# jwh97nn/AnyRef

Measured on AMD Instinct MI355X. Metric: images/sec (1024^2, 7B LLM+ViT-L+SAM-H), higher is better.
Workload: dtype bf16 (LLaMA / CLIP) + f16 (SAM encoder); 1 GPU; C2: LLaVA-7B + CLIP ViT-L/14 + SAM-H refer-seg forward, 1024x1024, S=320 prompt, 10 new tokens, KV cache; batch_per_gpu=1, global_batch=1, parallelism=dp1, weights=random-init N(0,0.02^2) rounded to bf16

## Files before the change

### anyref_amd/_lib.py

```python
from __future__ import annotations

import ctypes as C
import os

import torch

HERE = os.path.dirname(os.path.abspath(__file__))
LIB_PATH = os.path.join(HERE, "libanyref_hip.so")

ABI_VERSION = 2
F32, BF16, F16 = 0, 1, 2
MODE_PARITY, MODE_PERF, MODE_PERF_FP8W, MODE_PARITY16, MODE_PERF_F16 = 0, 1, 2, 3, 4


class AnyrefConfig(C.Structure):
    _fields_ = [
        ("abi_version", C.c_int32), ("mode", C.c_int32),
        ("clip_image", C.c_int32), ("clip_patch", C.c_int32), ("clip_dim", C.c_int32),
        ("clip_heads", C.c_int32), ("clip_layers_run", C.c_int32), ("clip_mlp", C.c_int32),
        ("clip_eps", C.c_float),
        ("llm_vocab", C.c_int32), ("llm_dim", C.c_int32), ("llm_heads", C.c_int32),
        ("llm_layers", C.c_int32), ("llm_mlp", C.c_int32), ("llm_max_seq", C.c_int32),
        ("llm_rms_eps", C.c_float), ("llm_rope_theta", C.c_float),
        ("sam_img", C.c_int32), ("sam_patch", C.c_int32), ("sam_dim", C.c_int32), ("sam_depth", C.c_int32),
# ... 36 lines not shown
    "anyref_set_overlap": (_I, [_P, _I]),
    "anyref_set_early_tail": (_I, [_P, _I]),
    "anyref_set_extra_event": (_I, [_P, _P]),
    "anyref_set_graphs": (_I, [_P, _I]),
    "anyref_set_side_share": (_I, [_P, _I, _I]),
    "anyref_profile_enable": (_I, [_P, _I]),
    "anyref_profile_config": (_I, [_P, C.c_char_p, _I]),
    "anyref_profile_collect": (_I, [_P]),
    "anyref_profile_calibrate": (_I, [_P, _P, C.POINTER(C.c_double)]),
    "anyref_profile_read": (_I, [_P, _I, C.c_char_p, _I, C.POINTER(C.c_double), C.POINTER(_L),
                                C.POINTER(C.c_double), C.POINTER(C.c_double)]),
    "anyref_stamps_enable": (_I, [_P, _I]),
    "anyref_stamps_collect": (_I, [_P, C.POINTER(_L)]),
    "anyref_stamps_dropped": (_I, [_P, C.POINTER(_L)]),
    "anyref_stamps_read": (_I, [_P, _L, C.c_char_p, _I, C.POINTER(C.c_double), C.POINTER(C.c_double),
                               C.POINTER(C.c_double), C.POINTER(_I)]),
    "anyref_stamps_spread": (_I, [_P, _L, C.POINTER(C.c_double), C.POINTER(C.c_double), C.POINTER(C.c_double)]),
    "anyref_device_bytes": (_L, [_P]),
    "anyref_mode_name": (C.c_char_p, [_P]),
    "anyref_inexact_weights": (_I, [_P, C.POINTER(_L)]),
    "anyref_op_gemm": (_I, [_I, _P, _P, _P, _P, _P, _P, _P, _I, _I, _I, _I, _I]),
    "anyref_op_gemm_fp8": (_I, [_P, _P, _P, _P, _P, _P, _P, _I, _I, _I, _I, _I]),
    "anyref_op_quant_fp8": (_I, [_P, _P, _I, _I, _P, _P]),
    "anyref_op_gemv_fp8": (_I, [_P, _P, _P, _F, _P, _P, _P, _P, _P, _P, _I, _I, _I]),
    "anyref_op_iou_counts": (_I, [_P, _P, _P, _I, _L, _P]),
    "anyref_op_avs_counts": (_I, [_P, _P, _P, _I, _L, _P, _I, _F, _P, _P]),
    "anyref_op_sam_preprocess": (_I, [_P, _P, _I, _I, _I, C.POINTER(C.c_float), C.POINTER(C.c_float), _P]),
    "anyref_op_pil_resample_u8": (_I, [_P, _P, _I, _I, _I, _P, _P, _I, _I, _P, _P, _I, _P, _P, _I]),
    "anyref_op_pool_ref_tokens": (_I, [_P, _P, _I, _I, _I, _I, _P]),
    "anyref_op_kaldi_fbank": (_I, [_P, _P, _I, _I, _I, _I, _I, C.c_float, _P, _I, _P, _P, _I, C.c_float, C.c_float, _P]),
    "anyref_op_clip_finish": (_I, [_P, _P, _I, _I, _I, _I, _I, _I, _I, C.POINTER(C.c_float), C.POINTER(C.c_float), _P]),
    "anyref_op_gemv": (_I, [_I, _P, _P, _P, _F, _P, _P, _P, _P, _P, _I, _I, _I, _I]),
    "anyref_op_gemv_xn": (_I, [_I, _P, _P, _P, _F, _P, _P, _P, _P, _P, _I, _I, _I, _I, _P, _P, _I]),
    "anyref_op_rope_table": (_I, [_I, _I, _F, _P]),
    "anyref_op_decode_attn": (_I, [_I, _P, _P, _I, _I, _I, _P, _P, _P, _P, _I, _F, _P, _P, _I]),
    "anyref_op_rope_cache": (_I, [_I, _P, _P, _P, _P, _I, _I, _I, _I, _P, _P, _P, _P, _P, _P, _I, _P]),
    "anyref_op_argmax": (_I, [_P, _P, _I, _I, _I, _P, _P, _P, _I, _I, _I, _P, _P, _P]),
    "anyref_op_norm": (_I, [_I, _P, _P, _P, _P, _P, _I, _I, _F, _I]),
    "anyref_op_attention": (_I, [_I, _P, _P, _P, _P, _P, _I, _I, _I, _I, _I, _F, _I, _P, _P, _P, _I, _I]),
    "anyref_op_attention_tab": (_I, [_I, _P, _P, _P, _P, _P, _I, _I, _I, _I, _F, _P, _P, _I, _I, _I]),
    "anyref_op_gemm_gather": (_I, [_I, _P, _P, _P, _P, _P, _P, _P, _I, _I, _I, _I]),
    "anyref_op_attention_relp": (_I, [_I, _P, _P, _P, _P, _P, _I, _I, _I, _I, _F, _P, _I, _I, _I]),
    "anyref_op_rel_pos": (_I, [_I, _P, _P, _P, _P, _I, _I, _I, _I, _P, _P]),
    "anyref_op_postprocess": (_I, [_P, _P, _I, _I, _I, _I, _I, _I, _I, _I, _P]),
    "anyref_op_last_error": (C.c_char_p, []),
}

_lib = None


def load() -> C.CDLL:
    global _lib
    if _lib is not None:
        return _lib
    if not os.path.exists(LIB_PATH):
        raise RuntimeError(
            f"{LIB_PATH} not found: build the HIP backend first "
            "(`python -c 'import __graft_entry__ as g; g.build()'` or `make -C anyref_amd/csrc`). "
            "anyref_amd has no CPU fallback.")
    lib = C.CDLL(LIB_PATH)
    for name, (res, args) in SYMBOLS.items():
        fn = getattr(lib, name)
        fn.restype = res
        fn.argtypes = args
    _lib = lib
    return lib
# ... 1 lines not shown
```

### anyref_amd/csrc/gemv.hip

```cpp
#include <cstdlib>
#include <stdexcept>
#include <type_traits>

#include "kernels.h"

namespace anyref {

static bool gemv_pair_knob() {
  static const bool p = !(getenv("ANYREF_GEMV_PAIR") && atoi(getenv("ANYREF_GEMV_PAIR")) == 0);
  return p;
}
static int gemv_grid_knob() {
  static const int g = getenv("ANYREF_GEMV_GRID") ? atoi(getenv("ANYREF_GEMV_GRID")) : 0;
  return g;
}

#ifndef ANYREF_GEMV_NO_DOT2
#define ANYREF_GEMV_NO_DOT2 0
#endif
constexpr bool NO_DOT2 = ANYREF_GEMV_NO_DOT2;
template <typename T, int NB, bool DUAL, int XPT, bool W8 = false, bool PAIR = false>
__global__ __launch_bounds__(512) void gemv_kernel(GemvArgs a, int b0, int nb) {
  static_assert(!W8 || std::is_same<T, bf16>::value, "fp8 weights go with bf16 activations");
  using WE = std::conditional_t<is_split<T>::value, bf16, T>;
  using XE = std::conditional_t<is_split<T>::value, float, T>;
  using WT = std::conditional_t<W8, uint8_t, WE>;
  constexpr int VN = W8 ? 16 : Vec16<WE>::N;
  constexpr int R = DUAL ? 1 : 2;
  constexpr int RW = 2;
  constexpr int UNR = 4;
  constexpr bool DOT2 = (std::is_same<T, bf16>::value || is_half16<T>::value) && !W8 && !NO_DOT2;
  extern __shared__ __attribute__((aligned(16))) char smem[];
  XE* xs = reinterpret_cast<XE*>(smem);
  __shared__ float red[NB][8];
  __shared__ float red2[2][4][2][NB];
  const int tid = threadIdx.x, lane = tid & 63, wave = tid >> 6;
  const int K = a.K;
  __shared__ unsigned long long st_t[2];
  __shared__ unsigned st_cnt;
  unsigned long long t_begin = 0;
  if (a.stamp.base) {
    t_begin = wall_clock64();
    if (tid == 0) {
      st_t[0] = ~0ull;
      st_t[1] = 0;
      st_cnt = 0;
    }
// ... 173 lines not shown
      const int n0 = (unit + (t / nchp) * nunits) * R;
#pragma unroll
      for (int r = 0; r < RW; ++r)
#pragma unroll
        for (int b = 0; b < NB; ++b) acc[r][b] = wave_sum(acc[r][b]);
      if constexpr (PAIR) {
        const int buf = (t / nchp) & 1;
        if (half == 1 && lane == 0) {
#pragma unroll
          for (int r = 0; r < RW; ++r)
#pragma unroll
            for (int b = 0; b < NB; ++b) red2[buf][wave >> 1][r][b] = acc[r][b];
        }
        __syncthreads();
        if (half == 0) {
#pragma unroll
          for (int r = 0; r < RW; ++r)
#pragma unroll
            for (int b = 0; b < NB; ++b) acc[r][b] += red2[buf][wave >> 1][r][b];
        }
      }
      if (lane < R * NB && half == 0) {
        const int r = lane / NB, b = lane % NB, n = n0 + r;
        float v = 0.f, v2 = 0.f;
#pragma unroll
        for (int rr = 0; rr < R; ++rr)
#pragma unroll
          for (int bb = 0; bb < NB; ++bb)
            if (lane == rr * NB + bb) {
              v = acc[rr][bb];
              v2 = DUAL ? acc[RW - 1][bb] : 0.f;
            }
        if (n < a.N && b < nb) {
          if constexpr (W8) {
            v *= a.wscale[(int64_t)n * a.ws_stride];
            if (DUAL) v2 *= a.wscale2[(int64_t)n * a.ws_stride];
          }
          if (a.bias) v += a.bias[n];
          if (DUAL)
            v = apply_act(v, ACT_SILU) * v2;
          else
            v = apply_act(v, a.act);
          const int64_t o = (int64_t)(b0 + b) * a.ldy + n;
          if (a.resid) v += a.resid[o];
          a.y[o] = v;
        }
      }
#pragma unroll
      for (int r = 0; r < RW; ++r)
#pragma unroll
        for (int b = 0; b < NB; ++b) acc[r][b] = 0.f;
    }
    if (t + 1 < items) {
#pragma unroll
      for (int u = 0; u < UNR; ++u)
#pragma unroll
        for (int r = 0; r < RW; ++r) wcur[u][r] = wnxt[u][r];
    }
  }
  if (a.stamp.base && lane == 0) {
    atomicMin(&st_t[0], t_begin);
    atomicMax(&st_t[1], (unsigned long long)wall_clock64());
    if (atomicAdd(&st_cnt, 1u) == 7u) {
      const int e = *a.stamp.epoch;
      if (e < a.stamp.max_epoch) {
        unsigned long long* p = a.stamp.base + (size_t)e * a.stamp.stride + (size_t)blockIdx.x * 2;
        p[0] = st_t[0];
        p[1] = st_t[1];
      }
    }
  }
}


template <bool W8, bool DUAL, int XV>
__global__ __launch_bounds__(512) void gemv_rows8_kernel(GemvArgs a, int b0, int nb, int kh0, int rs) {
  typedef __attribute__((ext_vector_type(2))) __bf16 bf16x2;
  constexpr int NB = 8, UNR = 8;
  constexpr int EPL = W8 ? 16 : 8;
  constexpr int SEG = 16 * EPL;
  constexpr int CH = UNR * SEG;
  using WT = std::conditional_t<W8, uint8_t, bf16>;
  extern __shared__ __attribute__((aligned(16))) char smem[];
  __shared__ float red[NB][8];
  const int tid = threadIdx.x, lane = tid & 63, wave = tid >> 6;
  const int j = lane & 3, q = lane >> 2;
  const int K = a.K;
  const int ldw = a.ldw > 0 ? a.ldw : K;
  const WT* __restrict__ W = reinterpret_cast<const WT*>(a.W);
  const WT* __restrict__ W2 = reinterpret_cast<const WT*>(a.W2);
  constexpr int R = DUAL ? 2 : 4;
  const int ngroups = cdiv(a.N, R);
  const int nwaves = gridDim.x * 8, gw = blockIdx.x * 8 + wave;
  const int my_groups = gw < ngroups ? (ngroups - gw + nwaves - 1) / nwaves : 0;
  const int nkh = kh0 < K ? 2 : 1;
  const int nch0 = cdiv(kh0, CH), nch1 = nkh == 2 ? cdiv(K - kh0, CH) : 0;
  const int items0 = my_groups * nch0, items = items0 + my_groups * nch1;
  const int pl = rs > 0 ? (rs - 64) / 2 : 0;
  uint4v w0[UNR], w1[UNR], w2[UNR];
  auto item_pos = [&](int t, int& g, int& kbeg, int& kend) __attribute__((always_inline)) {
    int gi, c;
    if (t < items0) {
      gi = t / nch0; c = t - gi * nch0;
      kbeg = c * CH; kend = kh0;
// ... 231 lines not shown
  const int rs = cdiv(kh0 * 2, 256) * 256 + 64;
  const size_t lds = (size_t)8 * rs;
  const int grid = 256;
  const double wbytes = (double)a.N * a.K * wsz * (dual ? 2 : 1) + (double)nb * (a.K + a.N) * 4;
  char tag[48];
  snprintf(tag, sizeof(tag), "gemv_rows8_%s%s", w8 ? "fp8w" : "bf16", dual ? "_swiglu" : "");
  ProfScope prof(tag, 2.0 * nb * a.N * (double)a.K * (dual ? 2 : 1), wbytes, s);
  auto launch = [&](auto w8_t, auto dual_t, auto xv_t) {
    constexpr bool W8 = decltype(w8_t)::value, DUAL = decltype(dual_t)::value;
    constexpr int XV = decltype(xv_t)::value;
    auto kern = &gemv_rows8_kernel<W8, DUAL, XV>;
    static KernelAttrOnce once;
    ensure_dyn_lds(once, reinterpret_cast<const void*>(kern), 152 * 1024);
    hipLaunchKernelGGL(kern, dim3(grid), dim3(512), lds, s, a, b0, nb, kh0, rs);
  };
  using TT = std::true_type;
  using FF = std::false_type;
  using X2 = std::integral_constant<int, 2>;
  using X3 = std::integral_constant<int, 3>;
  auto by_xv = [&](auto w8_t, auto dual_t) {
    if (a.gain && a.K > 4096) launch(w8_t, dual_t, X3());
    else launch(w8_t, dual_t, X2());
  };
  if (w8) {
    if (dual) by_xv(TT(), TT());
    else by_xv(TT(), FF());
  } else {
    if (dual) by_xv(FF(), TT());
    else by_xv(FF(), FF());
  }
  return true;
}

template <typename T, int NB>
static void gemv_dispatch(const GemvArgs& a_in, int b0, int nb, hipStream_t s) {
  GemvArgs a = a_in;
  const size_t lds = (size_t)NB * a.K * (is_split<T>::value ? 4 : sizeof(T));
  if (lds > 150 * 1024) throw std::runtime_error("gemv: K too large for the LDS activation stage");
  int grid = 256 * (lds > 76 * 1024 ? 1 : 2);
  const int grid_rule = grid;
  if (a.grid > 0 && a.grid < grid) grid = a.grid;
  if (gemv_grid_knob() > 0) grid = gemv_grid_knob();
  auto go = [&](auto xpt_tag) {
    constexpr int XPT = decltype(xpt_tag)::value;
    const double wsz = a.w_fp8 ? 1.0 : (is_split<T>::value ? 2.0 : (double)sizeof(T));
    const double wbytes = (double)a.N * a.K * wsz * (a.W2 ? 2 : 1) + (double)nb * (a.K + a.N) * 4;
    char tag[40];
    snprintf(tag, sizeof(tag), "gemv_%s%s_x%d",
             a.w_fp8 ? "fp8w" : (is_split<T>::value ? "sp16" : is_half16<T>::value ? "f16" : sizeof(T) == 2 ? "bf16" : "f32"),
             a.W2 ? "_swiglu" : "", XPT);
    ProfScope prof(tag, 2.0 * nb * a.N * (double)a.K * (a.W2 ? 2 : 1), wbytes, s);
    if (g_stamp && g_stamp->on) a.stamp = g_stamp->slot(tag, wbytes, grid);
    auto launch = [&](auto dual_t, auto w8_t, auto pair_t) {
      constexpr bool DUAL = decltype(dual_t)::value, W8 = decltype(w8_t)::value, PAIR = decltype(pair_t)::value;
      auto kern = &gemv_kernel<T, NB, DUAL, XPT, W8, PAIR>;
      static KernelAttrOnce once;
      ensure_dyn_lds(once, reinterpret_cast<const void*>(kern), 150 * 1024);
      hipLaunchKernelGGL(kern, dim3(grid), dim3(512), lds, s, a, b0, nb);
    };
    using TT = std::true_type;
    using FF = std::false_type;
    const bool pair = gemv_pair_knob() && cdiv(a.N, a.W2 ? 1 : 2) * 2 <= (gemv_grid_knob() > 0 ? grid : grid_rule) * 8;
    auto by_pair = [&](auto dual_t, auto w8_t) {
      if (pair) launch(dual_t, w8_t, TT());
      else launch(dual_t, w8_t, FF());
    };
    if constexpr (std::is_same<T, bf16>::value) {
      if (a.w_fp8) {
        if (a.W2) by_pair(TT(), TT());
        else by_pair(FF(), TT());
        return;
      }
    }
    if (a.W2) by_pair(TT(), FF());
    else by_pair(FF(), FF());
  };
  if (a.K <= 512 * 8)
    go(std::integral_constant<int, 8>());
  else if (a.K <= 512 * 24)
    go(std::integral_constant<int, 24>());
  else if (a.K <= 512 * 32)
    go(std::integral_constant<int, 32>());
  else
    throw std::runtime_error("gemv: K > 16384 not supported");
}

template <typename T>
void launch_gemv(const GemvArgs& a, hipStream_t s) {
  const int VN = a.w_fp8 ? 16 : Vec16<std::conditional_t<is_split<T>::value, bf16, T>>::N;
  if (a.K % VN || ((uintptr_t)a.W & 15)) throw std::runtime_error("gemv: K must be a multiple of 16 bytes");
  if (a.w_fp8 && (!std::is_same<T, bf16>::value || !a.wscale || (a.W2 && !a.wscale2)))
    throw std::runtime_error("gemv: fp8 weights need the bf16 mode and per-row scales");
  if (((uintptr_t)a.x & 15) || a.ldx % 4 || a.K % 4 || (a.gain && ((uintptr_t)a.gain & 15)) ||
      (a.xn_out && (((uintptr_t)a.xn_out & 15) || a.xn_ld % 4)))
    throw std::runtime_error("gemv: x / gain / xn_out rows must be 16-byte aligned");
// ... 47 lines not shown
```

### anyref_amd/csrc/kernels.h

```cpp
#pragma once
#include <cstdlib>
#include <map>
#include <string>
#include <utility>
#include <vector>

#include "common.h"

namespace anyref {

struct ProfStat {
  double ms = 0;
  int64_t count = 0;
  double flops = 0, bytes = 0;
};
class Profiler {
 public:
  ~Profiler();
  bool begin(const char* tag, double flops, double bytes, hipStream_t s);
  void end(hipStream_t s);
  void collect();
  void reset();
  void calibrate(hipStream_t s);
  double null_ms = 0.0;
// ... 99 lines not shown
  float* slabs_out = nullptr;
  int slabs = 0;
  bool* norm_done = nullptr;
  int batch = 1;
  int64_t sA = 0, sW = 0, sC = 0, sR = 0, sBias = 0;
};
template <typename T>
void launch_gemm(const GemmArgs& a, hipStream_t s);
void gemm_reserve_workspace(hipStream_t s, size_t bytes);
void gemm_release_workspace(hipStream_t s);
void attn_release_workspace(hipStream_t s);

struct GemvArgs {
  const float* x = nullptr;
  const float* gain = nullptr;
  float eps = 1e-6f;
  const void* W = nullptr;
  const void* W2 = nullptr;
  const float* bias = nullptr;
  float* y = nullptr;
  const float* resid = nullptr;
  int B = 1, N = 0, K = 0, ldx = 0, ldy = 0;
  int act = ACT_NONE;
  int ldw = 0;
  int w_fp8 = 0;
  const float* wscale = nullptr;
  const float* wscale2 = nullptr;
  int ws_stride = 1;
  float* xn_out = nullptr;
  const int* xn_row_map = nullptr;
  int xn_ld = 0;
  StampArgs stamp;
  int grid = 0;
};
template <typename T>
void launch_gemv(const GemvArgs& a, hipStream_t s);
void launch_gemv_skinny_f32(const GemvArgs& a, hipStream_t s);
void launch_quant_fp8_rows(const float* src, int lds, int N, int K, uint8_t* q, int ldq, float* scale, hipStream_t s,
                           int scale_stride = 1, unsigned long long* inexact = nullptr);
void launch_dequant_fp8_rows(const uint8_t* q, int ldq, const float* scale, int N, int K, void* out_bf16, int ldo,
                             hipStream_t s);

struct NormArgs {
  const float* x = nullptr;
  const float* gain = nullptr;
  const float* bias = nullptr;
  void* y = nullptr;
  const int* row_map = nullptr;
  int M = 0, D = 0, ldx = 0, ldy = 0;
  float eps = 1e-5f;
  int rms = 0;
  int y_f32 = 0;
  int act = ACT_NONE;
  void* fill_dst = nullptr;
  int fill_ld = 0, fill_n = 0, fill_N = 0;
  const int* fill_rows = nullptr;
  const float* fill_bias = nullptr;
  bool* fill_done = nullptr;
};
template <typename T>
void launch_norm(const NormArgs& a, hipStream_t s);

struct AttnArgs {
  const void *Q = nullptr, *K = nullptr, *V = nullptr;
  void* O = nullptr;
  int64_t q_bs = 0, q_rs = 0, q_hs = 0;
  int64_t k_bs = 0, k_rs = 0, k_hs = 0;
// ... 127 lines not shown
```

### anyref_amd/csrc/model.hip

```cpp
#include <algorithm>
#include <cmath>
#include <cstdlib>
#include <cstring>
#include <type_traits>

#include "model.h"

namespace anyref {

ModelBase::ModelBase(const anyref_config& c, int device) : cfg(c), device_(device) { HIP_TRY(hipSetDevice(device)); }

ModelBase::~ModelBase() {
  (void)hipSetDevice(device_);
  (void)hipDeviceSynchronize();
  for (auto& kv : allocs_) (void)hipFree(kv.first);
  if (wcount_) (void)hipFree(wcount_);
}

unsigned long long* ModelBase::weight_counts() {
  if (!wcount_) {
    HIP_TRY(hipMalloc(&wcount_, 2 * sizeof(unsigned long long)));
    HIP_TRY(hipMemset(wcount_, 0, 2 * sizeof(unsigned long long)));
  }
  return wcount_;
// ... 198 lines not shown
  bool gemm(hipStream_t s, const E* A, int lda, const Lin<typename ModeTypes<E>::W>& l, void* C, int ldc, int M, int act, bool c_f32,
            const float* resid = nullptr, int ldr = 0, const int* row_map = nullptr, const Affine* nrm = nullptr,
            void* nrm_out = nullptr, bool swiglu = false, float ln_eps = -1.f, const int* a_row_map = nullptr) {
    GemmArgs a;
    bool fused = false;
    a.swiglu_pairs = swiglu ? 1 : 0;
    if (nrm && nrm_out) {
      a.norm_gain = nrm->g; a.norm_out = nrm_out; a.norm_ld = l.n; a.norm_eps = cfg.llm_rms_eps; a.norm_done = &fused;
      if (ln_eps >= 0.f) {
        a.norm_bias = nrm->b;
        a.norm_eps = ln_eps;
      }
    }
    a.A = A; a.lda = apad<E>(lda); a.W = l.w; a.ldw = l.stride(); a.bias = l.b; a.C = C; a.ldc = c_f32 ? ldc : apad<E>(ldc);
    a.M = M; a.N = l.n;
    a.norm_ld = apad<E>(a.norm_ld);
    a.K = l.k; a.act = act; a.c_f32 = c_f32 ? 1 : 0; a.resid = resid; a.ldr = ldr; a.row_map = row_map;
    a.a_row_map = a_row_map;
    a.max_wg = cap_wg_;
    if constexpr (std::is_same<E, T>::value && !SPT) {
      if (l.w8) {
        if (l.k % 64 == 0) {
          a.W = l.w8; a.w_fp8 = 1; a.col_scale = l.ws;
        } else {
          launch_dequant_fp8_rows(l.w8, l.stride(), l.ws, l.n, l.k, deq_buf_, l.k, s);
          a.W = deq_buf_; a.ldw = l.k;
        }
      }
    }
    launch_gemm<E>(a, s);
    return fused;
  }
  int gemv_grid_ = 0;
  void gemv_w(GemvArgs& g, const Lin<W>& l, int row0 = 0) const {
    g.ldw = l.stride();
    g.grid = gemv_grid_;
    if (l.w8) {
      g.W = l.w8 + (size_t)row0 * l.stride();
      g.wscale = l.ws + row0;
      g.w_fp8 = 1;
    } else {
      g.W = l.w + (size_t)row0 * l.stride();
    }
  }
  void gemv_w2(GemvArgs& g, const Lin<W>& l, int row0) const {
    if (l.w8) {
      g.W2 = l.w8 + (size_t)row0 * l.stride();
      g.wscale2 = l.ws + row0;
    } else {
      g.W2 = l.w + (size_t)row0 * l.stride();
    }
  }
  static constexpr int kEmbDtype = std::is_same<W, bf16>::value ? 1 : is_half16<W>::value ? 2 : 0;
  bool fp8w_ = false;
  W* deq_buf_ = nullptr;
  void pack_rows_fp8(Lin<W>& l, int row0, const std::string& name, int rows, int cols, int rstride = 1) {
    const RawTensor& t = raw(name);
    if (t.numel() != (int64_t)rows * cols || cols != l.k)
      throw std::runtime_error("shape mismatch for " + name + " (fp8 pack)");
    launch_quant_fp8_rows(t.p, cols, rows, cols, l.w8 + (size_t)row0 * l.stride(), l.stride() * rstride, l.ws + row0, 0,
                          rstride, weight_counts());
  }
  Lin<W> alloc_fp8(int n, int k) {
    if (k % 16) throw std::runtime_error("fp8 weights need K % 16 == 0");
    Lin<W> l;
    l.n = n;
    l.k = k;
    l.ld = k + kRowPadBytes;
    l.w8 = reinterpret_cast<uint8_t*>(dalloc((size_t)n * l.ld));
// ... 736 lines not shown
  sam_enq_done_ = false;
  sam_next_blk_ = 0;
  sam_img_ = sam_images;
  sam_B_ = B;
  early_pending_.clear();
  if (!fed) sam_feed((int)sam_blocks_.size(), false);
}
template <typename T, typename TS>
void Model<T, TS>::sam_feed(int upto, bool capped) {
  const int nblk = (int)sam_blocks_.size();
  if (!sam_forked_ || sam_enq_done_) return;
  upto = std::min(upto, nblk);
  if (upto <= sam_next_blk_) return;
  cap_wg_ = capped ? side_cap_now_ : 0;
  try {
    sam_encoder(s2_, sam_img_, sam_B_, sam_emb_, sam_next_blk_, upto);
  } catch (...) {
    cap_wg_ = 0;
    throw;
  }
  cap_wg_ = 0;
  sam_next_blk_ = upto;
  if (upto == nblk) {
    HIP_TRY(hipEventRecord(ev_sam_, s2_));
    sam_enq_done_ = true;
    for (const PendingEarly& e : early_pending_) early_seg_run(e);
    early_pending_.clear();
  }
}

template <typename T, typename TS>
void Model<T, TS>::decode_step_graph(hipStream_t s, int B, bool keep_q, bool corun) {
  static const int corun_grid = getenv("ANYREF_GEMV_CORUN_GRID") ? atoi(getenv("ANYREF_GEMV_CORUN_GRID")) : 256;
  struct GridScope {
    int& g;
    ~GridScope() { g = 0; }
  } grid_scope{gemv_grid_};
  gemv_grid_ = corun ? corun_grid : 0;
  if (!use_graphs_ || (g_prof && g_prof->on)) {
    llm_decode_step(s, B, keep_q);
    return;
  }
  const bool stamped = stamp.on;
  const int key = B * 8 + (corun && corun_grid > 0 ? 4 : 0) + (keep_q ? 2 : 0) + (stamped ? 1 : 0);
  auto it = decode_graphs_.find(key);
  if (it == decode_graphs_.end()) {
    if (keep_q) ensure_q_last();
    if (!cap_stream_) HIP_TRY(hipStreamCreateWithFlags(&cap_stream_, hipStreamNonBlocking));
    gemm_reserve_workspace(cap_stream_, (size_t)8 * cfg.max_batch *
                                            std::max(std::max(3 * cfg.llm_dim, 2 * cfg.llm_mlp), cfg.llm_vocab) * 4);
    hipGraph_t g = nullptr;
    hipGraphExec_t ge = nullptr;
    HIP_TRY(hipStreamBeginCapture(cap_stream_, hipStreamCaptureModeRelaxed));
    try {
      if (stamped) stamp.graph_begin(key);
      llm_decode_step(cap_stream_, B, keep_q);
      if (stamped) stamp.graph_end(cap_stream_);
    } catch (...) {
      if (stamped) stamp.graph_abort();
      hipStreamEndCapture(cap_stream_, &g);
      if (g) hipGraphDestroy(g);
      throw;
    }
    HIP_TRY(hipStreamEndCapture(cap_stream_, &g));
    HIP_TRY(hipGraphInstantiate(&ge, g, nullptr, nullptr, 0));
    HIP_TRY(hipGraphDestroy(g));
    it = decode_graphs_.emplace(key, ge).first;
  }
  HIP_TRY(hipGraphLaunch(it->second, s));
  if (stamped) stamp.graph_replayed(key);
}
// ... 873 lines not shown
```

### anyref_amd/csrc/optest.hip

```cpp
#include <algorithm>
#include <string>
#include <vector>

#include "../../include/anyref_hip_ops.h"
#include "kernels.h"

using namespace anyref;

static thread_local std::string g_op_err;

#define OP_GUARD(body)                                   \
  try {                                                  \
    body;                                                \
    hipError_t _e = hipGetLastError();                   \
    if (_e != hipSuccess) {                              \
      g_op_err = std::string("HIP error: ") + hipGetErrorString(_e); \
      return 3;                                          \
    }                                                    \
    return 0;                                            \
  } catch (const std::exception& e) {                    \
    g_op_err = e.what();                                 \
    return 2;                                            \
  }

// ... 43 lines not shown
    else launch_gemm<bf16>(a, (hipStream_t)stream);
  });
}

int anyref_op_gemv(int t, void* stream, const float* x, const float* gain, float eps, const void* W,
                   const void* W2, const float* bias, float* y, const float* resid, int B, int N, int K, int act) {
  OP_GUARD({
    GemvArgs a;
    a.x = x; a.ldx = K; a.gain = gain; a.eps = eps; a.W = W; a.W2 = W2; a.bias = bias; a.y = y; a.resid = resid;
    a.ldy = N; a.B = B; a.N = N; a.K = K; a.act = act;
    if (const char* e = getenv("ANYREF_OPTEST_LDW_PAD")) a.ldw = K + atoi(e);
    if (t == 3) launch_gemv<sp16>(a, (hipStream_t)stream);
    else if (t == 0) launch_gemv<float>(a, (hipStream_t)stream);
    else if (t == 2) launch_gemv<f16>(a, (hipStream_t)stream);
    else launch_gemv<bf16>(a, (hipStream_t)stream);
  });
}

int anyref_op_gemv_xn(int t, void* stream, const float* x, const float* gain, float eps, const void* W, const void* W2,
                      const float* bias, float* y, const float* resid, int B, int N, int K, int act, float* xn_out,
                      const int32_t* xn_row_map, int xn_ld) {
  OP_GUARD({
    GemvArgs a;
    a.x = x; a.ldx = K; a.gain = gain; a.eps = eps; a.W = W; a.W2 = W2; a.bias = bias; a.y = y; a.resid = resid;
    a.ldy = N; a.B = B; a.N = N; a.K = K; a.act = act;
    a.xn_out = xn_out; a.xn_row_map = xn_row_map; a.xn_ld = xn_ld;
    if (t == 0) launch_gemv<float>(a, (hipStream_t)stream);
    else if (t == 1) launch_gemv<bf16>(a, (hipStream_t)stream);
    else if (t == 2) launch_gemv<f16>(a, (hipStream_t)stream);
    else throw std::runtime_error("op_gemv_xn: t = 0 / 1 / 2");
  });
}

int anyref_op_rope_table(int S, int hd, float theta, float* out_host) { OP_GUARD(rope_table(S, hd, theta, out_host)); }

int anyref_op_decode_attn(int t, void* stream, const float* qkv, int B, int H, int hd, const int32_t* pos,
                          const float* cs_tab, void* kc, void* vc, int maxS, float scale, float* out, void* q_keep,
                          int force_fallback) {
  OP_GUARD({
    if (t != 0 && t != 1 && t != 2) throw std::runtime_error("op_decode_attn: t = 0 / 1 / 2");
    hipStream_t st = (hipStream_t)stream;
    std::vector<int> h(B);
    HIP_TRY(hipMemcpy(h.data(), pos, (size_t)B * 4, hipMemcpyDeviceToHost));
    for (int& v : h) v += 1;
    TmpBuf kv_len((size_t)B * 4);
    TmpBuf q_tmp((size_t)B * H * hd * 4);
    HIP_TRY(hipMemcpy(kv_len.p, h.data(), (size_t)B * 4, hipMemcpyHostToDevice));
    if (t == 0)
      launch_decode_step_attn<float>(qkv, B, H, hd, pos, (const int*)kv_len.p, cs_tab, q_tmp.p, kc, vc, maxS, scale, out,
                                     q_keep, st, force_fallback != 0);
    else if (t == 2)
      launch_decode_step_attn<f16>(qkv, B, H, hd, pos, (const int*)kv_len.p, cs_tab, q_tmp.p, kc, vc, maxS, scale, out,
                                   q_keep, st, force_fallback != 0);
    else
      launch_decode_step_attn<bf16>(qkv, B, H, hd, pos, (const int*)kv_len.p, cs_tab, q_tmp.p, kc, vc, maxS, scale, out,
                                    q_keep, st, force_fallback != 0);
  });
}

int anyref_op_rope_cache(int t, void* stream, const void* qkv, const float* slab0, const float* slab1, int B, int S, int H,
                         int hd, const int32_t* pos0, const int32_t* lens, const float* cs_tab, void* q_out, void* kc,
                         void* vc, int maxS, void* q_keep) {
  OP_GUARD({
    hipStream_t st = (hipStream_t)stream;
    if (t != 0 && t != 1 && t != 2) throw std::runtime_error("op_rope_cache: t = 0 / 1 / 2");
    if (slab0) {
// ... 199 lines not shown
```

### include/anyref_hip_ops.h

```cpp
#ifndef ANYREF_HIP_OPS_H
#define ANYREF_HIP_OPS_H
#include <stdint.h>
#ifdef __cplusplus
extern "C" {
#endif

int anyref_op_gemm(int t, void* stream, const void* A, const void* W, const float* bias, void* C,
                   const float* resid, const int32_t* row_map, int M, int N, int K, int act, int c_f32);
int anyref_op_gemv(int t, void* stream, const float* x, const float* gain, float eps, const void* W,
                   const void* W2, const float* bias, float* y, const float* resid, int B, int N, int K, int act);
int anyref_op_gemv_xn(int t, void* stream, const float* x, const float* gain, float eps, const void* W, const void* W2,
                      const float* bias, float* y, const float* resid, int B, int N, int K, int act, float* xn_out,
                      const int32_t* xn_row_map, int xn_ld);
int anyref_op_rope_table(int S, int hd, float theta, float* out_host);
int anyref_op_decode_attn(int t, void* stream, const float* qkv, int B, int H, int hd, const int32_t* pos,
                          const float* cs_tab, void* kc, void* vc, int maxS, float scale, float* out, void* q_keep,
                          int force_fallback);
int anyref_op_rope_cache(int t, void* stream, const void* qkv, const float* slab0, const float* slab1, int B, int S, int H,
                         int hd, const int32_t* pos0, const int32_t* lens, const float* cs_tab, void* q_out, void* kc,
                         void* vc, int maxS, void* q_keep);
int anyref_op_argmax(void* stream, const float* x, int M, int N, int ldx, int64_t* out, int32_t* pos, const void* table,
                     int is_bf16, int D, int maxS, float* x_next, int32_t* row_map, int32_t* kvlen);
int anyref_op_norm(int t, void* stream, const float* x, const float* gain, const float* bias, float* y, int M,
                   int D, float eps, int rms);
int anyref_op_attention(int t, void* stream, const void* q, const void* k, const void* v, void* o, int B, int H,
                        int Sq, int Sk, int hd, float scale, int causal, const int32_t* kv_len,
                        const float* rel_h, const float* rel_w, int kh, int kw);
int anyref_op_rel_pos(int t, void* stream, const void* q, const float* tab_h, const float* tab_w, int B, int H,
                      int size, int hd, float* rel_h, float* rel_w);
int anyref_op_quant_fp8(void* stream, const float* src, int N, int K, uint8_t* q, float* scale);
int anyref_op_gemm_fp8(void* stream, const void* A, const uint8_t* W8, const float* scale, const float* bias, void* C,
                       const float* resid, int M, int N, int K, int act, int c_f32);
int anyref_op_gemv_fp8(void* stream, const float* x, const float* gain, float eps, const uint8_t* W,
                       const uint8_t* W2, const float* scale, const float* scale2, float* y, const float* resid,
                       int B, int N, int K);
int anyref_op_iou_counts(void* stream, const float* logits, const uint8_t* target, int n, int64_t hw,
                         int64_t* counts);
int anyref_op_avs_counts(void* stream, const float* logits, const uint8_t* target, int n, int64_t hw,
                         const float* cuts, int nth, float cut_pred, int64_t* conf, int64_t* hist);
int anyref_op_sam_preprocess(void* stream, const uint8_t* img, int h, int w, int S, const float* mean3,
                             const float* std3, float* out);
int anyref_op_pil_resample_u8(void* stream, const uint8_t* in, int H, int W, int C, uint8_t* tmp, uint8_t* out,
                              int ow, int oh, const int32_t* xbounds, const int32_t* xk, int kx,
                              const int32_t* ybounds, const int32_t* yk, int ky);
int anyref_op_pool_ref_tokens(void* stream, const float* feats, int n, int L, int H, int n_out, float* out);
int anyref_op_clip_finish(void* stream, const uint8_t* img, int ih, int iw, int y0, int x0, int h, int w, int S,
// ... 19 lines not shown
```

Measured before the change: 25.57 images/sec.

## Add LDS ring-buffered async-load GEMV for decode steps co-running with other work

Adds a new 16-bit weight GEMV kernel that streams weight tiles into a per-wave LDS ring using global_load_lds and waits with explicit vmcnt, keeping several loads in flight while computing dot products. It is used for batch-1 decode steps when the decode co-runs with other work (corun), on a smaller fixed grid, so each block hides memory latency without relying on high occupancy. Shared x-staging, output epilogue and timestamp code are factored into helpers. The change raises LDS use and adds inline-asm synchronisation complexity, and it only applies on the corun path.

```diff
diff --git a/anyref_amd/_lib.py b/anyref_amd/_lib.py
--- a/anyref_amd/_lib.py
+++ b/anyref_amd/_lib.py
@@ -92,6 +92,7 @@
     "anyref_op_clip_finish": (_I, [_P, _P, _I, _I, _I, _I, _I, _I, _I, C.POINTER(C.c_float), C.POINTER(C.c_float), _P]),
     "anyref_op_gemv": (_I, [_I, _P, _P, _P, _F, _P, _P, _P, _P, _P, _I, _I, _I, _I]),
     "anyref_op_gemv_xn": (_I, [_I, _P, _P, _P, _F, _P, _P, _P, _P, _P, _I, _I, _I, _I, _P, _P, _I]),
+    "anyref_op_gemv_ring": (_I, [_I, _P, _P, _P, _F, _P, _P, _P, _P, _P, _I, _I, _I, _P, _I, _I]),
     "anyref_op_rope_table": (_I, [_I, _I, _F, _P]),
     "anyref_op_decode_attn": (_I, [_I, _P, _P, _I, _I, _I, _P, _P, _P, _P, _I, _F, _P, _P, _I]),
     "anyref_op_rope_cache": (_I, [_I, _P, _P, _P, _P, _I, _I, _I, _I, _P, _P, _P, _P, _P, _P, _I, _P]),
diff --git a/anyref_amd/csrc/gemv.hip b/anyref_amd/csrc/gemv.hip
--- a/anyref_amd/csrc/gemv.hip
+++ b/anyref_amd/csrc/gemv.hip
@@ -13,6 +13,116 @@
 static int gemv_grid_knob() {
   static const int g = getenv("ANYREF_GEMV_GRID") ? atoi(getenv("ANYREF_GEMV_GRID")) : 0;
   return g;
+}
+static int gemv_ring_grid_knob() {
+  static const int g = getenv("ANYREF_GEMV_RING_GRID") ? atoi(getenv("ANYREF_GEMV_RING_GRID")) : 0;
+  return g;
+}
+
+template <typename XE, int NB, int XPT, typename FirstLoads, typename Sync>
+__device__ __forceinline__ void gemv_stage_x(const GemvArgs& a, int K, int b0, int nb, XE* xs, float (&red)[NB][8], int tid,
+                                             int lane, int wave, FirstLoads first_loads, Sync sync) {
+  if (!a.gain) {
+    constexpr int XV = (XPT + 3) / 4;
+    float4v xv[NB][XV];
+#pragma unroll
+    for (int b = 0; b < NB; ++b) {
+      const float* x = a.x + (int64_t)(b0 + (b < nb ? b : 0)) * a.ldx;
+#pragma unroll
+      for (int i = 0; i < XV; ++i) {
+        const int k = (tid + i * 512) * 4;
+        xv[b][i] = (b < nb && k < K) ? *reinterpret_cast<const float4v*>(x + k) : float4v{0.f, 0.f, 0.f, 0.f};
+      }
+    }
+    first_loads();
+#pragma unroll
+    for (int b = 0; b < NB; ++b) {
+      if (b >= nb) continue;
+#pragma unroll
+      for (int i = 0; i < XV; ++i) {
+        const int k = (tid + i * 512) * 4;
+        if (k < K) store4_from_f32<XE>(&xs[b * K + k], xv[b][i][0], xv[b][i][1], xv[b][i][2], xv[b][i][3]);
+      }
+    }
+  } else {
+    constexpr int XV = (XPT + 3) / 4;
+    float4v xr[NB][XV], gr[XV];
+#pragma unroll
+    for (int i = 0; i < XV; ++i) {
+      const int k = (tid + i * 512) * 4;
+      gr[i] = k < K ? *reinterpret_cast<const float4v*>(a.gain + k) : float4v{1.f, 1.f, 1.f, 1.f};
+    }
+#pragma unroll
+    for (int b = 0; b < NB; ++b) {
+      const float* x = a.x + (int64_t)(b0 + (b < nb ? b : 0)) * a.ldx;
+#pragma unroll
+      for (int i = 0; i < XV; ++i) {
+        const int k = (tid + i * 512) * 4;
+        xr[b][i] = (b < nb && k < K) ? *reinterpret_cast<const float4v*>(x + k) : float4v{0.f, 0.f, 0.f, 0.f};
+      }
+    }
+    first_loads();
+    float scale[NB];
+#pragma unroll
+    for (int b = 0; b < NB; ++b) {
+      float ss = 0.f;
+#pragma unroll
+      for (int i = 0; i < XV; ++i)
+#pragma unroll
+        for (int e = 0; e < 4; ++e) ss += xr[b][i][e] * xr[b][i][e];
+      ss = wave_sum(ss);
+      if (lane == 0) red[b][wave] = ss;
+    }
+    sync();
+#pragma unroll
+    for (int b = 0; b < NB; ++b) {
+      float tot = 0.f;
+#pragma unroll
+      for (int w = 0; w < 8; ++w) tot += red[b][w];
+      scale[b] = rsqrtf(tot / (float)K + a.eps);
+    }
+#pragma unroll
+    for (int b = 0; b < NB; ++b) {
+      if (b >= nb) continue;
+#pragma unroll
+      for (int i = 0; i < XV; ++i) {
+        const int k = (tid + i * 512) * 4;
+        if (k < K) {
+          const float4v v = xr[b][i] * scale[b] * gr[i];
+          store4_from_f32<XE>(&xs[b * K + k], v[0], v[1], v[2], v[3]);
+          if (a.xn_out && blockIdx.x == 0)
+            *reinterpret_cast<float4v*>(a.xn_out + (int64_t)(a.xn_row_map ? a.xn_row_map[b0 + b] : b0 + b) * a.xn_ld + k) = v;
+        }
+      }
+    }
+  }
+}
+
+template <bool DUAL, bool W8>
+__device__ __forceinline__ float gemv_out_value(const GemvArgs& a, int n, float v, float v2) {
+  if constexpr (W8) {
+    v *= a.wscale[(int64_t)n * a.ws_stride];
+    if (DUAL) v2 *= a.wscale2[(int64_t)n * a.ws_stride];
+  }
+  if (a.bias) v += a.bias[n];
+  if (DUAL)
+    v = apply_act(v, ACT_SILU) * v2;
+  else
+    v = apply_act(v, a.act);
+  return v;
+}
+__device__ __forceinline__ void gemv_stamp_end(const GemvArgs& a, unsigned long long (&st_t)[2], unsigned& st_cnt,
+                                               unsigned long long t_begin) {
+  atomicMin(&st_t[0], t_begin);
+  atomicMax(&st_t[1], (unsigned long long)wall_clock64());
+  if (atomicAdd(&st_cnt, 1u) == 7u) {
+    const int e = *a.stamp.epoch;
+    if (e < a.stamp.max_epoch) {
+      unsigned long long* p = a.stamp.base + (size_t)e * a.stamp.stride + (size_t)blockIdx.x * 2;
+      p[0] = st_t[0];
+      p[1] = st_t[1];
+    }
+  }
 }
 
 #ifndef ANYREF_GEMV_NO_DOT2
@@ -252,15 +362,7 @@
               v2 = DUAL ? acc[RW - 1][bb] : 0.f;
             }
         if (n < a.N && b < nb) {
-          if constexpr (W8) {
-            v *= a.wscale[(int64_t)n * a.ws_stride];
-            if (DUAL) v2 *= a.wscale2[(int64_t)n * a.ws_stride];
-          }
-          if (a.bias) v += a.bias[n];
-          if (DUAL)
-            v = apply_act(v, ACT_SILU) * v2;
-          else
-            v = apply_act(v, a.act);
+          v = gemv_out_value<DUAL, W8>(a, n, v, v2);
           const int64_t o = (int64_t)(b0 + b) * a.ldy + n;
           if (a.resid) v += a.resid[o];
           a.y[o] = v;
@@ -278,18 +380,7 @@
         for (int r = 0; r < RW; ++r) wcur[u][r] = wnxt[u][r];
     }
   }
-  if (a.stamp.base && lane == 0) {
-    atomicMin(&st_t[0], t_begin);
-    atomicMax(&st_t[1], (unsigned long long)wall_clock64());
-    if (atomicAdd(&st_cnt, 1u) == 7u) {
-      const int e = *a.stamp.epoch;
-      if (e < a.stamp.max_epoch) {
-        unsigned long long* p = a.stamp.base + (size_t)e * a.stamp.stride + (size_t)blockIdx.x * 2;
-        p[0] = st_t[0];
-        p[1] = st_t[1];
-      }
-    }
-  }
+  if (a.stamp.base && lane == 0) gemv_stamp_end(a, st_t, st_cnt, t_begin);
 }
 
 
@@ -587,6 +678,167 @@
   return true;
 }
 
+typedef const __attribute__((address_space(1))) void* gemv_gas_ptr;
+typedef __attribute__((address_space(3))) void* gemv_las_ptr;
+template <int N>
+__device__ __forceinline__ void gemv_wait_vmcnt() {
+  asm volatile("s_waitcnt vmcnt(%0)" ::"n"(N) : "memory");
+}
+__device__ __forceinline__ void gemv_ring_barrier() { asm volatile("s_waitcnt lgkmcnt(0)\n\ts_barrier" ::: "memory"); }
+__device__ __forceinline__ uint32_t gemv_lds_addr(const void* p) {
+  return (uint32_t)(uintptr_t)(gemv_las_ptr)(const_cast<void*>(p));
+}
+constexpr int GEMV_RING_S = 8;
+
+template <typename T, bool DUAL, int XPT, bool PAIR, int S>
+__global__ __launch_bounds__(512) void gemv_ring_kernel(GemvArgs a, int b0) {
+  static_assert(std::is_same<T, bf16>::value || is_half16<T>::value, "16-bit weights");
+  typedef __attribute__((ext_vector_type(2))) __bf16 bf16x2;
+  typedef __attribute__((ext_vector_type(2))) _Float16 f16x2;
+  constexpr int NB = 1, VN = 8, R = DUAL ? 1 : 2, RW = 2, UNR = 4, CH = 64 * VN * UNR;
+  constexpr int PIECE = 64 * 16;
+  extern __shared__ __attribute__((aligned(16))) char smem[];
+  T* xs = reinterpret_cast<T*>(smem);
+  __shared__ float red[NB][8];
+  __shared__ float red2[2][4][RW];
+  const int tid = threadIdx.x, lane = tid & 63, wave = tid >> 6;
+  const int K = a.K;
+  __shared__ unsigned long long st_t[2];
+  __shared__ unsigned st_cnt;
+  unsigned long long t_begin = 0;
+  if (a.stamp.base) {
+    t_begin = wall_clock64();
+    if (tid == 0) {
+      st_t[0] = ~0ull;
+      st_t[1] = 0;
+      st_cnt = 0;
+    }
+  }
+  const T* __restrict__ W = reinterpret_cast<const T*>(a.W);
+  const T* __restrict__ W2 = reinterpret_cast<const T*>(a.W2);
+  const int ldw = a.ldw > 0 ? a.ldw : K;
+  const int nwaves = gridDim.x * 8;
+  const int gw = blockIdx.x * 8 + wave;
+  const int ngroups = cdiv(a.N, R);
+  const int nch = cdiv(K, CH);
+  const int unit = PAIR ? gw >> 1 : gw, nunits = PAIR ? nwaves >> 1 : nwaves, half = PAIR ? (gw & 1) : 0;
+  const int nchp = PAIR ? (nch + 1) >> 1 : nch;
+  const int my_groups = PAIR ? cdiv(ngroups, nunits) : (gw < ngroups ? (ngroups - gw + nwaves - 1) / nwaves : 0);
+  const int items = my_groups * nchp;
+  const int P = items * UNR;
+  char* ring = smem + K * (int)sizeof(T) + wave * (S * RW * PIECE);
+
+  auto issue = [&](int p, int slot) __attribute__((always_inline)) {
+    const int t = p / UNR, u = p - t * UNR;
+    const int g = unit + (t / nchp) * nunits, c = PAIR ? 2 * (t % nchp) + half : t % nchp;
+    const bool live = !PAIR || (g < ngroups && c < nch);
+    const int k = c * CH + u * 64 * VN + lane * VN;
+    const int kk = live && k < K ? k : 0;
+    const int n0 = g * R;
+    char* dst = ring + slot * (RW * PIECE);
+#pragma unroll
+    for (int r = 0; r < RW; ++r) {
+      const T* src;
+      if (DUAL && r == RW - 1) {
+        src = W2 + (int64_t)(n0 < a.N ? n0 : a.N - 1) * ldw + kk;
+      } else {
+        const int n = n0 + r < a.N ? n0 + r : a.N - 1;
+        src = W + (int64_t)n * ldw + kk;
+      }
+      __builtin_amdgcn_global_load_lds((gemv_gas_ptr)src, (gemv_las_ptr)(dst + r * PIECE), 16, 0, 2 );
+    }
+  };
+  const bool pre = a.resid && my_groups * R <= 64;
+  float rv = 0.f;
+  if (pre && lane < my_groups * R) {
+    const int n = (unit + (lane / R) * nunits) * R + lane % R;
+    if (n < a.N) rv = a.resid[(int64_t)b0 * a.ldy + n];
+  }
+  gemv_stage_x<T, NB, XPT>(a, K, b0, 1, xs, red, tid, lane, wave,
+                           [&]() {
+#pragma unroll
+                             for (int p = 0; p < S; ++p)
+                               if (p < P) issue(p, p);
+                           },
+                           []() { gemv_ring_barrier(); });
+  gemv_ring_barrier();
+  asm volatile("" ::"v"(rv));
+
+  float acc[RW];
+#pragma unroll
+  for (int r = 0; r < RW; ++r) acc[r] = 0.f;
+  for (int t = 0; t < items; ++t) {
+    const int gi = t / nchp, ci = t - gi * nchp, c = PAIR ? 2 * ci + half : ci;
+    const bool live = !PAIR || (unit + gi * nunits < ngroups && c < nch);
+#pragma unroll
+    for (int u = 0; u < UNR; ++u) {
+      const int p = t * UNR + u, slot = p % S;
+      if (p + S - 1 < P) gemv_wait_vmcnt<(S - 1) * RW>();
+      else gemv_wait_vmcnt<0>();
+      const int k = c * CH + u * 64 * VN + lane * VN;
+      const char* sl = ring + slot * (RW * PIECE) + lane * 16;
+      uint4v w0, w1, xv;
+      asm volatile("ds_read_b128 %0, %3\n\tds_read_b128 %1, %4\n\tds_read_b128 %2, %5\n\ts_waitcnt lgkmcnt(0)"
+                   : "=&v"(w0), "=&v"(w1), "=&v"(xv)
+                   : "v"(gemv_lds_addr(sl)), "v"(gemv_lds_addr(sl + PIECE)), "v"(gemv_lds_addr(xs + (k < K ? k : 0)))
+                   : "memory");
+      if (p + S < P && !(a.ring_drop && slot == S - 1)) issue(p + S, slot);
+      if (live && k < K) {
+        const uint4v wv[RW] = {w0, w1};
+#pragma unroll
+        for (int r = 0; r < RW; ++r)
+#pragma unroll
+          for (int j = 0; j < 4; ++j) {
+            const uint32_t wj = wv[r][j], xj = xv[j];
+            if constexpr (is_half16<T>::value)
+              acc[r] = __builtin_amdgcn_fdot2(__builtin_bit_cast(f16x2, wj), __builtin_bit_cast(f16x2, xj), acc[r], false);
+            else
+              acc[r] = __builtin_amdgcn_fdot2_f32_bf16(__builtin_bit_cast(bf16x2, wj), __builtin_bit_cast(bf16x2, xj),
+                                                       acc[r], false);
+          }
+      }
+    }
+    if (ci == nchp - 1) {
+      const int n0 = (unit + gi * nunits) * R;
+#pragma unroll
+      for (int r = 0; r < RW; ++r) acc[r] = wave_sum(acc[r]);
+      if constexpr (PAIR) {
+        const int buf = gi & 1;
+        if (half == 1 && lane == 0) {
+#pragma unroll
+          for (int r = 0; r < RW; ++r) red2[buf][wave >> 1][r] = acc[r];
+        }
+        gemv_ring_barrier();
+        if (half == 0) {
+#pragma unroll
+          for (int r = 0; r < RW; ++r) acc[r] += red2[buf][wave >> 1][r];
+        }
+      }
+      const float rg = __shfl(rv, gi * R + (lane < R ? lane : 0), 64);
+      if (lane < R && half == 0) {
+        const int n = n0 + lane;
+        float v = 0.f, v2 = 0.f;
+#pragma unroll
+        for (int rr = 0; rr < R; ++rr)
+          if (lane == rr) {
+            v = acc[rr];
+            v2 = DUAL ? acc[RW - 1] : 0.f;
+          }
+        if (n < a.N) {
+          v = gemv_out_value<DUAL, false>(a, n, v, v2);
+          const int64_t o = (int64_t)b0 * a.ldy + n;
+          if (a.resid) v += pre ? rg : a.resid[o];
+          a.y[o] = v;
+        }
+      }
+#pragma unroll
+      for (int r = 0; r < RW; ++r) acc[r] = 0.f;
+    }
+  }
+  gemv_wait_vmcnt<0>();
+  if (a.stamp.base && lane == 0) gemv_stamp_end(a, st_t, st_cnt, t_begin);
+}
+
 template <typename T, int NB>
 static void gemv_dispatch(const GemvArgs& a_in, int b0, int nb, hipStream_t s) {
   GemvArgs a = a_in;
@@ -600,6 +852,34 @@
     constexpr int XPT = decltype(xpt_tag)::value;
     const double wsz = a.w_fp8 ? 1.0 : (is_split<T>::value ? 2.0 : (double)sizeof(T));
     const double wbytes = (double)a.N * a.K * wsz * (a.W2 ? 2 : 1) + (double)nb * (a.K + a.N) * 4;
+    const bool pair = gemv_pair_knob() && cdiv(a.N, a.W2 ? 1 : 2) * 2 <= (gemv_grid_knob() > 0 ? grid : grid_rule) * 8;
+    if constexpr (NB == 1 && (std::is_same<T, bf16>::value || is_half16<T>::value)) {
+      const size_t ring_lds = lds + (size_t)8 * GEMV_RING_S * 2 * 1024;
+      if (a.ring > 0 && !a.w_fp8 && nb == 1 && ring_lds <= 156 * 1024) {
+        const int rgrid = gemv_ring_grid_knob() > 0 ? gemv_ring_grid_knob() : a.ring;
+        char rtag[48];
+        snprintf(rtag, sizeof(rtag), "gemv_%s_ring%s_x%d", is_half16<T>::value ? "f16" : "bf16", a.W2 ? "_swiglu" : "", XPT);
+        ProfScope prof(rtag, 2.0 * a.N * (double)a.K * (a.W2 ? 2 : 1), wbytes, s);
+        if (g_stamp && g_stamp->on) a.stamp = g_stamp->slot(rtag, wbytes, rgrid);
+        auto launch = [&](auto dual_t, auto pair_t) {
+          constexpr bool DUAL = decltype(dual_t)::value, PAIR = decltype(pair_t)::value;
+          auto kern = &gemv_ring_kernel<T, DUAL, XPT, PAIR, GEMV_RING_S>;
+          static KernelAttrOnce once;
+          ensure_dyn_lds(once, reinterpret_cast<const void*>(kern), 156 * 1024);
+          hipLaunchKernelGGL(kern, dim3(rgrid), dim3(512), ring_lds, s, a, b0);
+        };
+        using RT = std::true_type;
+        using RF = std::false_type;
+        if (a.W2) {
+          if (pair) launch(RT(), RT());
+          else launch(RT(), RF());
+        } else {
+          if (pair) launch(RF(), RT());
+          else launch(RF(), RF());
+        }
+        return;
+      }
+    }
     char tag[40];
     snprintf(tag, sizeof(tag), "gemv_%s%s_x%d",
              a.w_fp8 ? "fp8w" : (is_split<T>::value ? "sp16" : is_half16<T>::value ? "f16" : sizeof(T) == 2 ? "bf16" : "f32"),
@@ -615,7 +895,6 @@
     };
     using TT = std::true_type;
     using FF = std::false_type;
-    const bool pair = gemv_pair_knob() && cdiv(a.N, a.W2 ? 1 : 2) * 2 <= (gemv_grid_knob() > 0 ? grid : grid_rule) * 8;
     auto by_pair = [&](auto dual_t, auto w8_t) {
       if (pair) launch(dual_t, w8_t, TT());
       else launch(dual_t, w8_t, FF());
diff --git a/anyref_amd/csrc/kernels.h b/anyref_amd/csrc/kernels.h
--- a/anyref_amd/csrc/kernels.h
+++ b/anyref_amd/csrc/kernels.h
@@ -155,7 +155,10 @@
   int xn_ld = 0;
   StampArgs stamp;
   int grid = 0;
-};
+  int ring = 0;
+  int ring_drop = 0;
+};
+constexpr int GEMV_RING_GRID = 128;
 template <typename T>
 void launch_gemv(const GemvArgs& a, hipStream_t s);
 void launch_gemv_skinny_f32(const GemvArgs& a, hipStream_t s);
diff --git a/anyref_amd/csrc/model.hip b/anyref_amd/csrc/model.hip
--- a/anyref_amd/csrc/model.hip
+++ b/anyref_amd/csrc/model.hip
@@ -254,9 +254,11 @@
     return fused;
   }
   int gemv_grid_ = 0;
+  int gemv_ring_ = 0;
   void gemv_w(GemvArgs& g, const Lin<W>& l, int row0 = 0) const {
     g.ldw = l.stride();
     g.grid = gemv_grid_;
+    g.ring = gemv_ring_;
     if (l.w8) {
       g.W = l.w8 + (size_t)row0 * l.stride();
       g.wscale = l.ws + row0;
@@ -1059,11 +1061,14 @@
 template <typename T, typename TS>
 void Model<T, TS>::decode_step_graph(hipStream_t s, int B, bool keep_q, bool corun) {
   static const int corun_grid = getenv("ANYREF_GEMV_CORUN_GRID") ? atoi(getenv("ANYREF_GEMV_CORUN_GRID")) : 256;
+  static const bool ring_on = !(getenv("ANYREF_GEMV_RING") && atoi(getenv("ANYREF_GEMV_RING")) == 0);
   struct GridScope {
     int& g;
-    ~GridScope() { g = 0; }
-  } grid_scope{gemv_grid_};
+    int& r;
+    ~GridScope() { g = r = 0; }
+  } grid_scope{gemv_grid_, gemv_ring_};
   gemv_grid_ = corun ? corun_grid : 0;
+  gemv_ring_ = corun && ring_on ? GEMV_RING_GRID : 0;
   if (!use_graphs_ || (g_prof && g_prof->on)) {
     llm_decode_step(s, B, keep_q);
     return;
diff --git a/anyref_amd/csrc/optest.hip b/anyref_amd/csrc/optest.hip
--- a/anyref_amd/csrc/optest.hip
+++ b/anyref_amd/csrc/optest.hip
@@ -99,6 +99,21 @@
   });
 }
 
+int anyref_op_gemv_ring(int t, void* stream, const float* x, const float* gain, float eps, const void* W, const void* W2,
+                        const float* bias, float* y, const float* resid, int N, int K, int act, float* xn_out, int grid,
+                        int drop) {
+  OP_GUARD({
+    GemvArgs a;
+    a.x = x; a.ldx = K; a.gain = gain; a.eps = eps; a.W = W; a.W2 = W2; a.bias = bias; a.y = y; a.resid = resid;
+    a.ldy = N; a.B = 1; a.N = N; a.K = K; a.act = act;
+    a.xn_out = xn_out; a.xn_ld = K;
+    a.ring = grid > 0 ? grid : GEMV_RING_GRID; a.ring_drop = drop;
+    if (t == 1) launch_gemv<bf16>(a, (hipStream_t)stream);
+    else if (t == 2) launch_gemv<f16>(a, (hipStream_t)stream);
+    else throw std::runtime_error("op_gemv_ring: t = 1 / 2");
+  });
+}
+
 int anyref_op_rope_table(int S, int hd, float theta, float* out_host) { OP_GUARD(rope_table(S, hd, theta, out_host)); }
 
 int anyref_op_decode_attn(int t, void* stream, const float* qkv, int B, int H, int hd, const int32_t* pos,
diff --git a/include/anyref_hip_ops.h b/include/anyref_hip_ops.h
--- a/include/anyref_hip_ops.h
+++ b/include/anyref_hip_ops.h
@@ -12,6 +12,9 @@
 int anyref_op_gemv_xn(int t, void* stream, const float* x, const float* gain, float eps, const void* W, const void* W2,
                       const float* bias, float* y, const float* resid, int B, int N, int K, int act, float* xn_out,
                       const int32_t* xn_row_map, int xn_ld);
+int anyref_op_gemv_ring(int t, void* stream, const float* x, const float* gain, float eps, const void* W, const void* W2,
+                        const float* bias, float* y, const float* resid, int N, int K, int act, float* xn_out, int grid,
+                        int drop);
 int anyref_op_rope_table(int S, int hd, float theta, float* out_host);
 int anyref_op_decode_attn(int t, void* stream, const float* qkv, int B, int H, int hd, const int32_t* pos,
                           const float* cs_tab, void* kc, void* vc, int maxS, float scale, float* out, void* q_keep,
```

After: 24.67 images/sec, median of 2. 0.965x the previous value.
